# meyerls/FruitNeRF

Measured on AMD Instinct MI355X. Metric: train rays/sec, fruit_nerf on synthetic apple 800x800, higher is better.
Workload: dtype f32 fwd (MLP GEMMs: 3-piece bf16 split, 6 products, ~2^-24) / 2-piece bwd (dX, dW: 3 products, ~2^-17; its forward recompute 3-piece); everything else f32

## Files before the change

fruitnerf_amd/csrc/field_bf16.hpp:

```cpp
#pragma once
#include "field_layers.hpp"

namespace fnr {

using bf16x8 = __attribute__((ext_vector_type(8))) __bf16;
using f32x8 = __attribute__((ext_vector_type(8))) float;

enum { MLP_FP32 = 0, MLP_BF16 = 1, MLP_BF16X3 = 3 };

template <class Cfg>
struct BfImage {
  static constexpr int NL = Cfg::NLAYERS;
  static constexpr int nib_used(int l) { return l == Cfg::L_COL0 ? Cfg::HB : Cfg::nib(l); }
  static constexpr int nkb(int l) { return (nib_used(l) + 1) / 2; }
  static constexpr int nkbT(int l) { return (Cfg::nob(l) + 1) / 2; }
  static constexpr bool hasT(int l) { return l != Cfg::L_SEM0; }
  static constexpr int fblocks(int l) { return Cfg::nob(l) * nkb(l); }
  static constexpr int tblocks(int l) { return hasT(l) ? nib_used(l) * nkbT(l) : 0; }
  static constexpr int foff(int l) {
    int o = 0;
    for (int i = 0; i < l; ++i) o += fblocks(i);
    return o;
  }
  static constexpr int F_TOTAL = foff(NL);
// ... 87 lines not shown
    pack_field_weights_block<Cfg>(p, packed, b);
    return;
  }
  b -= nb_pack;
  if (b < nb_pack16) {
    pack_field_weights_bf16_block<Cfg>(p, ns, image, b);
    return;
  }
  b -= nb_pack16;
  color_ray_bias_block<Cfg, true>(p, nullptr, rays, embedding, mean_embedding, ray_bias, b,
                                  (int)gridDim.x - nb_pack - nb_pack16);
}
template <class Cfg>
static inline void launch_prepare_field(const FieldPtrs& p, float* packed, int ns, __bf16* image, const RaysDev& rays,
                                        const float* embedding, const float* mean_embedding, float* ray_bias,
                                        hipStream_t st) {
  const int nb_pack = pack_field_weights_blocks<Cfg>();
  const int nb_pack16 = ns > 0 ? pack_field_weights_bf16_blocks<Cfg>() : 0;
  const long long nb_bias = color_ray_bias_blocks(rays);
  hipLaunchKernelGGL((k_prepare_field<Cfg>), dim3((unsigned)(nb_pack + nb_pack16 + nb_bias)), dim3(256), 0, st, p, packed, ns,
                     image, rays, embedding, mean_embedding, ray_bias, nb_pack, nb_pack16);
}

template <class Cfg, class Segs, int NS>
struct BfLds {
  using Img = BfImage<Cfg>;
  static constexpr int blocks(int s) { return Segs::isT(s) ? Img::tblocks(Segs::layer(s)) : Img::fblocks(Segs::layer(s)); }
  static constexpr int off(int s) {
    int o = 0;
    for (int i = 0; i < s; ++i) o += blocks(i) * NS;
    return o;
  }
  static constexpr int FRAGS = off(Segs::N);
  static constexpr int BYTES = FRAGS * 1024;
  static constexpr int find(int layer, bool isT) {
    for (int i = 0; i < Segs::N; ++i)
      if (Segs::layer(i) == layer && Segs::isT(i) == isT) return i;
    return -1;
  }
  template <int LAYER, bool IS_T>
  __device__ static __forceinline__ const bf16x8* seg(const bf16x8* lds) {
    constexpr int s = find(LAYER, IS_T);
    static_assert(s >= 0, "layer not staged by this kernel");
    return lds + off(s) * 64;
  }
  template <int LAYER, bool IS_T>
  static constexpr int seg_blocks() { return blocks(find(LAYER, IS_T)); }
  static constexpr int chunk_begin(int c) { return off(c / NS) * 64 + (c % NS) * blocks(c / NS) * 64; }
  static constexpr long long chunk_src(int c) {
    const int s = c / NS, pc = c % NS;
    return (long long)pc * Img::BLOCKS * 64 + (Segs::isT(s) ? Img::toff(Segs::layer(s)) : Img::foff(Segs::layer(s))) * 64;
  }
  template <int THREADS>
  __device__ static __forceinline__ void stage(bf16x8* __restrict__ lds, const __bf16* __restrict__ image) {
    constexpr int T = FRAGS * 64, NCH = Segs::N * NS;
    constexpr int PER = (T + THREADS - 1) / THREADS;
    static_assert(PER <= 32, "staging batch too large");
    const f32x4* img = reinterpret_cast<const f32x4*>(image);
    f32x4* dst = reinterpret_cast<f32x4*>(lds);
    f32x4 v[PER];
#pragma unroll
    for (int u = 0; u < PER; ++u) {
      const int f = (int)threadIdx.x + u * THREADS;
      long long delta = chunk_src(0) - chunk_begin(0);
#pragma unroll
      for (int c = 1; c < NCH; ++c) delta = (f >= chunk_begin(c)) ? chunk_src(c) - chunk_begin(c) : delta;
      if (f < T) v[u] = img[f + delta];
    }
#pragma unroll
    for (int u = 0; u < PER; ++u) {
      const int f = (int)threadIdx.x + u * THREADS;
      if (f < T) dst[f] = v[u];
    }
  }
};

template <class Cfg, int L, int NS, int THREADS>
__device__ __forceinline__ void bf_build_T(bf16x8* __restrict__ lds, const float* __restrict__ packed) {
  constexpr int NIB = Cfg::nib(L), NKT = (Cfg::nob(L) + 1) / 2, TB = NIB * NKT;
  for (int idx = threadIdx.x; idx < TB * 64; idx += THREADS) {
    const int blk = idx >> 6, lane = idx & 63;
    const int i = lane & 15, g = lane >> 4;
    const int kb = blk % NKT, ib = blk / NKT;
    float w[8];
#pragma unroll
    for (int e = 0; e < 8; ++e) {
      const int ob = 2 * kb + (e >> 2), row = 4 * g + (e & 3);
      w[e] = ob < Cfg::nob(L) ? packed[Cfg::woff(L) + ((ob * NIB + ib) * 64 + swz_slot(row, i >> 2)) * 4 + (i & 3)] : 0.0f;
    }
#pragma unroll
    for (int pc = 0; pc < NS; ++pc) {
      bf16x8 v;
#pragma unroll
      for (int e = 0; e < 8; ++e) v[e] = bf_piece(w[e], pc);
      lds[pc * TB * 64 + idx] = v;
    }
  }
}

using bf_f32x2 = __attribute__((ext_vector_type(2))) float;
using bf_bf16x2 = __attribute__((ext_vector_type(2))) __bf16;
__device__ __forceinline__ unsigned cvt_pk_bf16(float lo, float hi) {
  const bf_f32x2 v = {lo, hi};
  return __builtin_bit_cast(unsigned, __builtin_convertvector(v, bf_bf16x2));
}
using bf_u32x4 = __attribute__((ext_vector_type(4))) unsigned;
template <int NS>
__device__ __forceinline__ void bf_split(const f32x8 v, bf16x8 (&p)[NS]) {
  bf_u32x4 out[NS];
#pragma unroll
  for (int d = 0; d < 4; ++d) {
    float a = v[2 * d], b = v[2 * d + 1];
#pragma unroll
    for (int pc = 0; pc < NS; ++pc) {
      const unsigned w = cvt_pk_bf16(a, b);
      out[pc][d] = w;
      if (pc + 1 < NS) {
        a -= __builtin_bit_cast(float, w << 16);
        b -= __builtin_bit_cast(float, w & 0xffff0000u);
      }
    }
  }
#pragma unroll
  for (int pc = 0; pc < NS; ++pc) p[pc] = __builtin_bit_cast(bf16x8, out[pc]);
}
template <int NS>
// ... 101 lines not shown
#pragma unroll
    for (int s = NS - 1; s >= 0; --s)
#pragma unroll
      for (int pw = 0; pw <= s; ++pw)
        o[ob] = __builtin_amdgcn_mfma_f32_16x16x32_bf16(w[t & 1][pw], x[kb][s - pw], o[ob], 0, 0, 0);
    __builtin_amdgcn_sched_barrier(0);
  }
}
template <int NS, int NOB, int NIB>
__device__ __forceinline__ void bf_layer1(const bf16x8* __restrict__ seg, const float* __restrict__ B,
                                          const f32x4 (&in)[NIB], f32x4 (&o)[NOB], int lane) {
  const int g = lane >> 4;
#pragma unroll
  for (int ob = 0; ob < NOB; ++ob) o[ob] = *reinterpret_cast<const f32x4*>(B + 16 * ob + 4 * g);
  bf16x8 x[(NIB + 1) / 2][NS];
  bf_operand<NS, NIB>(in, x);
  bf_layer_acc1<NS, NOB, (NIB + 1) / 2>(seg, x, o, lane);
}
template <int NS, int NIBO, int NOB>
__device__ __forceinline__ void bf_layer_T1(const bf16x8* __restrict__ segT, const f32x4 (&G)[NOB], f32x4 (&o)[NIBO],
                                            int lane) {
#pragma unroll
  for (int ib = 0; ib < NIBO; ++ib) o[ib] = f32x4{0.f, 0.f, 0.f, 0.f};
  bf16x8 x[(NOB + 1) / 2][NS];
  bf_operand<NS, NOB>(G, x);
  bf_layer_acc1<NS, NIBO, (NOB + 1) / 2>(segT, x, o, lane);
}

size_t field_bf16_image_bytes();
int field_mlp_fwd_bf16(int cfg, int mode, const FieldPtrs& p, const float* packed, void* image_ws, const float* ray_bias,
                       const RaysDev& rd, int S, long long N, const float2* feats, const uint8_t* selector, float* density,
                       float* rgb, float* logit, float* geo_out, float* h_buf, hipStream_t st);
int field_mlp_fwd_sem_big_bf16(int mode, const FieldPtrs& p, void* image_ws, const float* packed, long long N,
                               const float* h_buf, float* logit, hipStream_t st);
int field_mlp_bwd_sem_big_bf16(int mode, const FieldPtrs& p, void* image_ws, const float* packed, long long N,
                               const float* h_saved, const float* d_logit, float* partials, long long blocks,
                               hipStream_t st, float* d_h_semgrad = nullptr);
namespace pw {
struct BwdArgs {
  const float* packed;
  const __bf16* image;
  const float* ray_bias;
  RaysDev rd;
  int S;
  long long N;
  const float2* feats;
  const float* h_saved;
  const uint8_t* selector;
  const float *d_density, *d_rgb, *d_logit;
  float2* d_feats;
  float *d_h, *gsum_tile, *gsum_extra, *partials;
  long long blocks;
  hipStream_t st;
};
}
int field_mlp_bwd_pw(int cfg, int mode, int branch, const pw::BwdArgs& a, const float2* jac, float4* d_pos);

}
```

fruitnerf_amd/csrc/field_layers.hpp:

```cpp
#pragma once
#include "common.hpp"

namespace fnr {

using f32x4 = __attribute__((ext_vector_type(4))) float;

enum KMap : int { KM_LINEAR = 0, KM_HASH = 1, KM_GEO = 2, KM_COLOR = 3 };

struct FieldCfgBase {
  static constexpr int GEO = 15, HB = 1, NSEM = 2, SEMB = 4;
  static constexpr int NLAYERS = 8;
  enum { L_BASE0 = 0, L_BASE1 = 1, L_SEM0 = 2, L_SEM1 = 3, L_SEM2 = -1, L_HEAD = 4, L_COL0 = 5, L_COL1 = 6, L_COL2 = 7 };
  static constexpr int nob(int l) { constexpr int a[NLAYERS] = {4, 1, 4, 4, 1, 4, 4, 1}; return a[l]; }
  static constexpr int nib(int l) { constexpr int a[NLAYERS] = {2, 4, 1, 4, 4, 4, 4, 4}; return a[l]; }
  static constexpr int out_dim(int l) { constexpr int a[NLAYERS] = {64, 16, 64, 64, 1, 64, 64, 3}; return a[l]; }
  static constexpr int in_dim(int l) { constexpr int a[NLAYERS] = {32, 64, 15, 64, 64, 63, 64, 64}; return a[l]; }
  static constexpr int km(int l) {
    constexpr int a[NLAYERS] = {KM_HASH, KM_LINEAR, KM_GEO, KM_LINEAR, KM_LINEAR, KM_COLOR, KM_LINEAR, KM_LINEAR};
    return a[l];
  }
  static constexpr int woff(int l) {
    int o = 0;
    for (int i = 0; i < l; ++i) o += nob(i) * nib(i) * 256;
    return o;
// ... 252 lines not shown
  float b;
  if constexpr (FROM_RAW) {
    constexpr int IN = Cfg::in_dim(Cfg::L_COL0);
    for (int i = threadIdx.x; i < COLOR_CONST_K * 64; i += 256) {
      const int o = i / COLOR_CONST_K, k = i - o * COLOR_CONST_K;
      Wt[k][o] = p.w[Cfg::L_COL0][o * IN + color_const_col<Cfg>(k)];
    }
    b = p.b[Cfg::L_COL0][lane];
  } else {
    const float* src = packed + Cfg::LDS_FLOATS;
    for (int i = threadIdx.x; i < COLOR_CONST_K * 64; i += 256) Wt[i >> 6][i & 63] = src[i];
    b = packed[Cfg::W_TOTAL + Cfg::boff(Cfg::L_COL0) + lane];
  }
  __syncthreads();
  for (long long ray = (long long)block * 4 + wave; ray < rays.n_rays; ray += (long long)n_blocks * 4) {
    float c[16];
    sh16_all(rays.directions + 3 * ray, c);
    const float* emb = mean_embedding ? mean_embedding : embedding + (size_t)rays.cam[ray] * 32;
    float e[32];
#pragma unroll
    for (int k = 0; k < 32; k += 4) {
      const f32x4 v = *reinterpret_cast<const f32x4*>(emb + k);
      e[k] = v[0], e[k + 1] = v[1], e[k + 2] = v[2], e[k + 3] = v[3];
    }
    float acc = b;
#pragma unroll
    for (int k = 0; k < 16; ++k) acc = fmaf(Wt[k][lane], c[k], acc);
#pragma unroll
    for (int k = 0; k < 32; ++k) acc = fmaf(Wt[16 + k][lane], e[k], acc);
    ray_bias[(size_t)ray * 64 + lane] = acc;
  }
}
template <class Cfg>
__global__ __launch_bounds__(256) void k_color_ray_bias(const float* __restrict__ packed, RaysDev rays,
                                                        const float* __restrict__ embedding,
                                                        const float* __restrict__ mean_embedding,
                                                        float* __restrict__ ray_bias) {
  FieldPtrs none{};
  color_ray_bias_block<Cfg, false>(none, packed, rays, embedding, mean_embedding, ray_bias, blockIdx.x, gridDim.x);
}
static inline long long color_ray_bias_blocks(const RaysDev& rays) {
  long long blocks = (rays.n_rays + 7) / 8;
  if (blocks > 8ll * device_cu_count()) blocks = 8ll * device_cu_count();
  return blocks < 1 ? 1 : blocks;
}

template <class Cfg>
static inline void launch_color_ray_bias(const float* packed, const RaysDev& rays, const float* embedding,
                                         const float* mean_embedding, float* ray_bias, hipStream_t st) {
  hipLaunchKernelGGL((k_color_ray_bias<Cfg>), dim3((unsigned)color_ray_bias_blocks(rays)), dim3(256), 0, st, packed, rays,
                     embedding, mean_embedding, ray_bias);
}

}
```

fruitnerf_amd/csrc/field_mlp_bwd.hip:

```cpp
#include "field_layers.hpp"
#include "field_bf16.hpp"
#include "sequencer.hpp"

namespace fnr {

enum { BR_COLOR = 0, BR_SEM = 1, BR_BASE = 2, BR_SEM_A = 3, BR_SEM_B = 4 };

constexpr int SCR_LD = 20;
constexpr int SCR_FLOATS = 2 * 64 * SCR_LD;

__device__ __forceinline__ void wave_lds_fence() {
  __builtin_amdgcn_s_waitcnt(0xc07f);
  __builtin_amdgcn_wave_barrier();
  asm volatile("" ::: "memory");
  __builtin_amdgcn_sched_barrier(0);
}

template <int NOB, int NIB_TOTAL, int IB0, int NIBO>
__device__ __forceinline__ void mlp_layer_T(const float* __restrict__ P, const f32x4 (&G)[NOB], f32x4 (&out)[NIBO],
                                            int lane) {
  const int ip = lane & 15, kg = lane >> 4;
  const int a = ip >> 2, b = ip & 3;
  constexpr int QC = (NIBO > 2) ? 2 : NIBO;
  static_assert(NIBO % QC == 0, "input blocks must split evenly");
// ... 557 lines not shown
    for (; b + 7 * RD_Y < nblocks; b += 8 * RD_Y) {
      float v[8];
#pragma unroll
      for (int u = 0; u < 8; ++u) v[u] = partials[(size_t)(b + u * RD_Y) * TOT + idx];
#pragma unroll
      for (int u = 0; u < 8; ++u) s += v[u];
    }
    for (; b < nblocks; b += RD_Y) s += partials[(size_t)b * TOT + idx];
  }
  s_part[y][t] = s;
  __syncthreads();
  if (y != 0 || idx >= TOT) return;
#pragma unroll
  for (int q = 1; q < RD_Y; ++q) s += s_part[q][t];
  if (!ADAM && s == 0.0f) return;
  if (idx < Cfg::W_TOTAL) {
    int l = 0;
#pragma unroll
    for (int q = 1; q < Cfg::NLAYERS; ++q)
      if (idx >= Cfg::woff(q)) l = q;
    const int local = idx - Cfg::woff(l);
    const int r = local & 3, slot = (local >> 2) & 63, blk = local >> 8;
    const int nib = Cfg::nib(l);
    const int ib = blk % nib, ob = blk / nib;
    const int g = slot >> 4, i = (slot & 15) ^ g;
    const int out = 16 * ob + i;
    const int col = kmap<Cfg>(Cfg::km(l), ib, g, r, Cfg::in_dim(l));
    if (out < Cfg::out_dim(l) && col >= 0) {
      float* dst = const_cast<float*>(grads.w[l]) + out * Cfg::in_dim(l) + col;
      if constexpr (ADAM) weight_adam_entry(wa, dst, s);
      else *dst += s;
    }
  } else {
    const int bi = idx - Cfg::W_TOTAL;
    int l = 0;
#pragma unroll
    for (int q = 1; q < Cfg::NLAYERS; ++q)
      if (bi >= Cfg::boff(q)) l = q;
    const int o = bi - Cfg::boff(l);
    if (o < Cfg::out_dim(l)) {
      float* dst = const_cast<float*>(grads.b[l]) + o;
      if constexpr (ADAM) weight_adam_entry(wa, dst, s);
      else *dst += s;
    }
  }
}

template <class Cfg, bool ADAM>
__global__ __launch_bounds__(RD_IDX * RD_Y) void k_reduce_dw(const float* __restrict__ partials, int nblocks, FieldPtrs grads,
                                                             WeightAdam wa) {
  reduce_dw_block<Cfg, ADAM>((int)blockIdx.x, partials, nblocks, grads, wa);
}

constexpr int RAYG_RB = 16;
template <class Cfg>
__global__ __launch_bounds__(256) void k_color_ray_grads(RaysDev rays, int S, long long N,
                                                         const float* __restrict__ embedding,
                                                         const float* __restrict__ gsum_tile,
                                                         const float* __restrict__ gsum_extra,
                                                         float* __restrict__ g_ray, float* __restrict__ partials) {
  __shared__ float Gs[RAYG_RB][64];
  __shared__ __attribute__((aligned(16))) float Cs[RAYG_RB][COLOR_CONST_K];
  const int t = threadIdx.x, o = t & 63, kq = t >> 6;
  const long long R = rays.n_rays;
  f32x4 acc[3];
  float accb = 0.0f;
#pragma unroll
  for (int q = 0; q < 3; ++q) acc[q] = f32x4{0.f, 0.f, 0.f, 0.f};
  for (long long base = (long long)blockIdx.x * RAYG_RB; base < R; base += (long long)gridDim.x * RAYG_RB) {
#pragma unroll
    for (int i = 0; i < RAYG_RB / 4; ++i) {
      const int rr = kq + 4 * i;
      const long long ray = base + rr;
      float v = 0.0f;
      if (ray < R) {
        const long long s_lo = ray * S, s_hi = s_lo + S;
        for (long long tl = s_lo >> 4; tl <= (s_hi - 1) >> 4; ++tl) {
          const long long first = 16 * tl, last = (16 * tl + 15 < N) ? 16 * tl + 15 : N - 1;
          if (first >= s_lo && last < s_hi) v += gsum_tile[(size_t)tl * 64 + o];
        }
        if (gsum_extra) v += gsum_extra[(size_t)ray * 64 + o];
        g_ray[(size_t)ray * 64 + o] = v;
      }
      Gs[rr][o] = v;
    }
#pragma unroll
    for (int u = 0; u < RAYG_RB * COLOR_CONST_K / 256; ++u) {
      const int idx = t + 256 * u;
      const int rr = idx / COLOR_CONST_K, k = idx - rr * COLOR_CONST_K;
      const long long ray = base + rr;
      float v = 0.0f;
      if (ray < R) {
        if (k < 16) {
          float c[16];
          sh16_all(rays.directions + 3 * ray, c);
#pragma unroll
          for (int q = 0; q < 16; ++q) v = (k == q) ? c[q] : v;
        } else {
          v = embedding[(size_t)rays.cam[ray] * 32 + (k - 16)];
        }
      }
      Cs[rr][k] = v;
    }
    __syncthreads();
#pragma unroll
    for (int rr = 0; rr < RAYG_RB; ++rr) {
      const float gv = Gs[rr][o];
      const f32x4* cr = reinterpret_cast<const f32x4*>(&Cs[rr][12 * kq]);
#pragma unroll
      for (int q = 0; q < 3; ++q) {
        const f32x4 cv = cr[q];
#pragma unroll
        for (int e = 0; e < 4; ++e) acc[q][e] = fmaf(gv, cv[e], acc[q][e]);
      }
      accb += gv;
    }
    __syncthreads();
  }
  float* part = partials + (size_t)blockIdx.x * (Cfg::W_TOTAL + Cfg::B_TOTAL);
  const int ob = o >> 4, i = o & 15;
  constexpr int NIB0 = Cfg::HB + 3;
#pragma unroll
  for (int q = 0; q < 12; ++q) {
    const int k = 12 * kq + q, ib = Cfg::HB + (k >> 4), kk = k & 15;
    part[Cfg::woff(Cfg::L_COL0) + ((ob * NIB0 + ib) * 64 + swz_slot(i, kk >> 2)) * 4 + (kk & 3)] = acc[q >> 2][q & 3];
  }
  if (kq == 0) part[Cfg::W_TOTAL + Cfg::boff(Cfg::L_COL0) + o] = accb;
}
static_assert(RAYG_RB * COLOR_CONST_K % 256 == 0, "staging loop covers the batch exactly");

template <class Cfg, bool ADAM>
__device__ __forceinline__ void embedding_grad_block(int c, const RaysDev& rays, const float* __restrict__ g_ray,
                                                     const float* __restrict__ packed, float* __restrict__ g_embedding,
                                                     const WeightAdam& wa) {
  __shared__ float red[16][64];
  const int lane = threadIdx.x & 63, wave = threadIdx.x >> 6;
  float acc = 0.0f;
  for (long long base = 64 * wave; base < rays.n_rays; base += 1024) {
    const long long r = base + lane;
    unsigned long long match = __ballot(r < rays.n_rays && rays.cam[r] == c);
    while (match) {
      const int bit = __builtin_ctzll(match);
      match &= match - 1;
      acc += g_ray[(size_t)(base + bit) * 64 + lane];
    }
  }
  red[wave][lane] = acc;
  __syncthreads();
  if (threadIdx.x < 64) {
    float s = 0.0f;
#pragma unroll
    for (int w = 0; w < 16; ++w) s += red[w][lane];
    red[0][lane] = s;
  }
  __syncthreads();
  const int k = threadIdx.x >> 5, oo = threadIdx.x & 31;
  const float* Wt = packed + Cfg::LDS_FLOATS + (16 + k) * 64;
  float s = fmaf(Wt[oo], red[0][oo], Wt[oo + 32] * red[0][oo + 32]);
#pragma unroll
  for (int m = 16; m >= 1; m >>= 1) s += __shfl_xor(s, m, 64);
  if constexpr (ADAM) {
    if (oo == 0) weight_adam_entry(wa, g_embedding + (size_t)c * 32 + k, s);
  } else {
    if (oo == 0 && s != 0.0f) g_embedding[(size_t)c * 32 + k] += s;
  }
}

template <class Cfg, bool ADAM>
__global__ __launch_bounds__(1024) void k_embedding_grad(RaysDev rays, const float* __restrict__ g_ray,
                                                         const float* __restrict__ packed,
                                                         float* __restrict__ g_embedding, WeightAdam wa) {
  embedding_grad_block<Cfg, ADAM>((int)blockIdx.x, rays, g_ray, packed, g_embedding, wa);
}

static_assert(RD_IDX * RD_Y == 1024, "k_finish_weights: both roles are 1024-thread workgroups");
template <class Cfg, bool ADAM>
__global__ __launch_bounds__(1024) void k_finish_weights(int n_images, RaysDev rays, const float* __restrict__ g_ray,
                                                         const float* __restrict__ packed, float* __restrict__ g_embedding,
                                                         const float* __restrict__ partials, int nblocks, FieldPtrs grads,
                                                         WeightAdam wa) {
  if ((int)blockIdx.x < n_images) embedding_grad_block<Cfg, ADAM>((int)blockIdx.x, rays, g_ray, packed, g_embedding, wa);
  else reduce_dw_block<Cfg, ADAM>((int)blockIdx.x - n_images, partials, nblocks, grads, wa);
// ... 37 lines not shown

template <class Cfg>
int field_mlp_bwd_launch(const FieldPtrs& p, const FieldPtrs& gp, const fnr_field_net* net, const fnr_field_net* grads,
                         const RaysDev& rd, int S, long long N, const float* feats, const float* h_saved,
                         const float* ray_bias_saved, const float* packed_saved, const uint8_t* selector,
                         const float* d_density, const float* d_rgb, const float* d_logit, float* d_feats,
                         const BwdWorkspace& ws, hipStream_t st, const float* jacobian = nullptr,
                         float* d_position = nullptr, const WeightAdam* wadam = nullptr, bool semgrad = false) {
  const float2* jac = reinterpret_cast<const float2*>(jacobian);
  float4* d_pos = reinterpret_cast<float4*>(d_position);
  const long long n_tiles = (N + 15) / 16;
  const long long max_blocks = device_cu_count();
  float* partials = ws.partials;
  float* packed = ws.packed;
  float* gsum_extra = (S % 16 != 0) ? ws.gsum_extra : nullptr;
  const float2* f2 = reinterpret_cast<const float2*>(feats);
  float2* df2 = reinterpret_cast<float2*>(d_feats);
  void* bf16_image = ws.bf16_image;
  if (packed_saved) {
    packed = const_cast<float*>(packed_saved);
    bf16_image = reinterpret_cast<char*>(packed) + field_fwd_ws_image_offset();
  } else {
    launch_pack_field_weights<Cfg>(p, packed, st);
    FNR_LAUNCH_CHECK();
  }
  const float* ray_bias = ray_bias_saved;
  if (!ray_bias) {
    launch_color_ray_bias<Cfg>(packed, rd, net->embedding, nullptr, ws.ray_bias, st);
    FNR_LAUNCH_CHECK();
    ray_bias = ws.ray_bias;
  }
  if (gsum_extra) FNR_HIP(hipMemsetAsync(gsum_extra, 0, (size_t)rd.n_rays * 64 * sizeof(float), st));
  long long blocks = (n_tiles + 3) / 4;
  if (blocks > max_blocks) blocks = max_blocks;
  const dim3 grid((unsigned)blocks);
  const int mode = net->mlp_mode;
  constexpr int cfg_id = Cfg::NSEM == 2 ? 0 : 1;
  const bool bf_all = mode != FNR_MLP_FP32;
  const bool bf_sem_big = mode != FNR_MLP_FP32 && Cfg::NSEM == 3;
  const pw::BwdArgs bf{packed, reinterpret_cast<const __bf16*>(bf16_image), ray_bias, rd, S, N, f2, h_saved, selector, d_density,
                       d_rgb, d_logit, df2, ws.d_h, ws.gsum_tile, gsum_extra, partials, blocks, st};
  if (bf_all) {
    if (!packed_saved) {
      launch_pack_field_weights_bf16<Cfg>(p, mode == FNR_MLP_BF16 ? 1 : 3, reinterpret_cast<__bf16*>(bf16_image), st);
      FNR_LAUNCH_CHECK();
    }
    const int rc = field_mlp_bwd_pw(cfg_id, mode, 0, bf, nullptr, nullptr);
    if (rc) return rc;
  } else {
    hipLaunchKernelGGL((k_field_mlp_bwd_color<Cfg, 8>), grid, dim3(512), 0, st, packed, ray_bias, rd, S, N, h_saved, d_rgb,
                       ws.d_h, ws.gsum_tile, gsum_extra, partials);
  }
  FNR_LAUNCH_CHECK();
  {
    long long rb = (rd.n_rays + RAYG_RB - 1) / RAYG_RB;
    if (rb > blocks) rb = blocks;
    hipLaunchKernelGGL((k_color_ray_grads<Cfg>), dim3((unsigned)rb), dim3(256), 0, st, rd, S, N, net->embedding,
                       ws.gsum_tile, gsum_extra, ws.g_ray, partials);
    FNR_LAUNCH_CHECK();
  }
  if (bf_sem_big) {
    int rc = field_mlp_bwd_sem_big_bf16(mode, p, bf16_image, packed, N, h_saved, d_logit, partials, blocks, st,
                                        semgrad ? ws.d_h : nullptr);
    if (rc) return rc;
    rc = field_mlp_bwd_pw(cfg_id, mode, 2, bf, jac, d_pos);
    if (rc) return rc;
  } else if (bf_all) {
    int rc = semgrad ? field_mlp_bwd_pw(cfg_id, mode, 3, bf, nullptr, nullptr) : FNR_OK;
    if (rc) return rc;
    rc = field_mlp_bwd_pw(cfg_id, mode, 1, bf, nullptr, nullptr);
    if (rc) return rc;
    rc = field_mlp_bwd_pw(cfg_id, mode, 2, bf, jac, d_pos);
    if (rc) return rc;
  } else if constexpr (Cfg::NSEM == 2) {
    if (semgrad)
      hipLaunchKernelGGL((k_field_mlp_bwd_sem<Cfg, 8, true, float*>), grid, dim3(512), 0, st, packed, N, h_saved, d_logit,
                         partials, ws.d_h);
    else
      hipLaunchKernelGGL((k_field_mlp_bwd_sem<Cfg, 8>), grid, dim3(512), 0, st, packed, N, h_saved, d_logit, partials);
    FNR_LAUNCH_CHECK();
  } else {
    if (semgrad)
      hipLaunchKernelGGL((k_field_mlp_bwd_sem_big<Cfg, true, 4, true, float*>), grid, dim3(256), 0, st, packed, N, h_saved,
                         d_logit, partials, ws.d_h);
    else
      hipLaunchKernelGGL((k_field_mlp_bwd_sem_big<Cfg, true, 4>), grid, dim3(256), 0, st, packed, N, h_saved, d_logit,
                         partials);
    FNR_LAUNCH_CHECK();
    hipLaunchKernelGGL((k_field_mlp_bwd_sem_big<Cfg, false, 4>), grid, dim3(256), 0, st, packed, N, h_saved, d_logit,
                       partials);
    FNR_LAUNCH_CHECK();
  }
  if (!bf_all) {
    hipLaunchKernelGGL((k_field_mlp_bwd_base<Cfg, 8>), grid, dim3(512), 0, st, packed, N, f2, selector, d_density, ws.d_h,
                       df2, partials);
    FNR_LAUNCH_CHECK();
  }
  constexpr int TOT = Cfg::W_TOTAL + Cfg::B_TOTAL;
  const unsigned finish_blocks = (unsigned)net->n_images + (unsigned)((TOT + RD_IDX - 1) / RD_IDX);
  if (wadam)
    hipLaunchKernelGGL((k_finish_weights<Cfg, true>), dim3(finish_blocks), dim3(1024), 0, st, (int)net->n_images, rd, ws.g_ray,
                       packed, grads->embedding, partials, (int)blocks, gp, *wadam);
  else
    hipLaunchKernelGGL((k_finish_weights<Cfg, false>), dim3(finish_blocks), dim3(1024), 0, st, (int)net->n_images, rd,
                       ws.g_ray, packed, grads->embedding, partials, (int)blocks, gp, WeightAdam{});
  FNR_LAUNCH_CHECK();
  if (jac && d_pos && !bf_all) return position_contract(N, net->grid.n_levels, jac, df2, d_pos, st);
  return FNR_OK;
}
}

extern "C" size_t fnr_field_mlp_bwd_workspace_bytes(int64_t n_rays, int S) {
  if (n_rays < 0 || S <= 0) return 0;
  return bwd_workspace(nullptr, n_rays, S).bytes;
}

static int field_mlp_bwd_entry(const fnr_field_net* net, const fnr_field_net* grads, const fnr_rays* rays, int S,
                                 const float* feats, const float* h_saved, const float* ray_bias_saved,
                                 const float* packed_saved, const uint8_t* selector, const float* d_density, const float* d_rgb, const float* d_logit, float* d_feats,
                                 void* workspace, size_t workspace_bytes, void* stream, const float* jacobian,
                               float* d_position, const fnr_table_adam* weight_adam = nullptr,
                               const float* grad_arena = nullptr, bool semgrad = false) {
  WeightAdam wa{};
// ... 109 lines not shown
```

fruitnerf_amd/csrc/field_mlp_bwd_pw.hip:

```cpp
#include <type_traits>

#include "field_bf16.hpp"

namespace fnr {
namespace pw {

using s16x4 = __attribute__((ext_vector_type(4))) short;
using s16x8 = __attribute__((ext_vector_type(8))) short;
using u32x4 = __attribute__((ext_vector_type(4))) unsigned;
typedef s16x4 __attribute__((address_space(3))) lds_s16x4;

constexpr int TILE_BYTES = 512;
template <int NS, int NT>
constexpr int scratch_bytes() { return 4 * NS * NT * TILE_BYTES; }

template <int NT, int NB>
struct Acts {
  f32x4 v[NT][NB];
};
template <int NT, int NB, int NS>
struct Ops {
  bf16x8 v[NT][(NB + 1) / 2][NS];
};
template <int NT, int NB, int NS>
// ... 465 lines not shown
          const int ray = first_ray[t] + (j - col);
#pragma unroll
          for (int ob = 0; ob < 4; ++ob)
#pragma unroll
            for (int r = 0; r < 4; ++r) atomicAdd(&gsum_extra[(size_t)ray * 64 + 16 * ob + 4 * g + r], rs[0][ob][r]);
        }
      }
    }
    Acts<NT, HB> Gh;
    layer<NT, NS, HB, 4>(T::template seg<LC0, true>(wt), nullptr, g1, Gh, lane);
#pragma unroll
    for (int t = 0; t < NT; ++t)
      if (sm.ok[t]) {
#pragma unroll
        for (int hb = 0; hb < HB; ++hb) *reinterpret_cast<f32x4*>(d_h + (size_t)sm.n[t] * (16 * HB) + 16 * hb + 4 * g) = Gh.v[t][hb];
      }
  }
  const int lane = lane0;
  float* part = partials + (size_t)blockIdx.x * (Cfg::W_TOTAL + Cfg::B_TOTAL);
  constexpr int NA = 4 * HB, NALL = NA + 25;
  struct Table {
    __device__ static __forceinline__ Dest get(int b) {
      constexpr int NA = 4 * Cfg::HB;
      if (b < NA) return Dest{Cfg::woff(LC0), b / Cfg::HB, b % Cfg::HB, Cfg::HB + 3, 0};
      b -= NA;
      if (b < 16) return Dest{Cfg::woff(LC1), b >> 2, b & 3, 4, 0};
      if (b < 20) return Dest{Cfg::woff(LC2), 0, b - 16, 4, 0};
      if (b < 24) return Dest{Cfg::W_TOTAL + Cfg::boff(LC1), b - 20, 0, 0, 1};
      return Dest{Cfg::W_TOTAL + Cfg::boff(LC2), 0, 0, 0, 1};
    }
  };
  f32x4 all[NALL];
#pragma unroll
  for (int i = 0; i < NA; ++i) all[i] = accA[i];
#pragma unroll
  for (int i = 0; i < 16; ++i) all[NA + i] = accB[i];
#pragma unroll
  for (int i = 0; i < 4; ++i) all[NA + 16 + i] = accC[i];
#pragma unroll
  for (int i = 0; i < 4; ++i) all[NA + 20 + i] = bias_total(bB[i]);
  all[NA + 24] = bias_total(bC[0]);
  reduce_and_store<NALL, WAVES, Table>(smem, part, all, wave, lane);
  constexpr int NIB0 = Cfg::HB + 3;
  for (int i = threadIdx.x; i < 4 * 3 * 256; i += THREADS) {
    const int blk = i >> 8, ob = blk / 3, ib = Cfg::HB + blk % 3;
    part[Cfg::woff(LC0) + (ob * NIB0 + ib) * 256 + (i & 255)] = 0.0f;
  }
  for (int i = threadIdx.x; i < 64; i += THREADS) part[Cfg::W_TOTAL + Cfg::boff(LC0) + i] = 0.0f;
}

template <class Cfg, int NSF, int NS, int NT, int WAVES>
__global__ __launch_bounds__(64 * WAVES, WAVES / 4) void k_field_mlp_bwd_sem_pw(
    const float* __restrict__ packed, const __bf16* __restrict__ image, int N, const float* __restrict__ h_saved,
    const float* __restrict__ d_logit, float* __restrict__ partials) {
  static_assert(Cfg::NSEM == 2 && Cfg::HB == 1, "`fruit_nerf` shape");
  constexpr int THREADS = 64 * WAVES;
  constexpr int LS0 = Cfg::L_SEM0, LS1 = Cfg::L_SEM1, LH = Cfg::L_HEAD;
  static_assert(LS1 == LS0 + 1 && LH == LS1 + 1, "the branch's layers are adjacent in the fp32 image");
  using L = Lds<Cfg, SegsSemF<Cfg>, SegsSemT<Cfg>, NSF, NS, NT, WAVES, 128>;
  using F = typename L::F;
  using T = typename L::T;
  extern __shared__ __attribute__((aligned(16))) unsigned char smem[];
  bf16x8* wf = reinterpret_cast<bf16x8*>(smem);
  bf16x8* wt = reinterpret_cast<bf16x8*>(smem + F::BYTES);
  float* fbias = reinterpret_cast<float*>(smem + L::FB_OFF);
  F::template stage<THREADS>(wf, image);
  T::template stage<THREADS>(wt, image);
  for (int i = threadIdx.x; i < 128; i += THREADS) fbias[i] = packed[Cfg::W_TOTAL + Cfg::boff(LS0) + i];
  __syncthreads();
  const int lane0 = threadIdx.x & 63, wave = threadIdx.x >> 6;
  unsigned char* scr = smem + L::SCR_OFF + wave * scratch_bytes<NS, NT>();
  f32x4 accH[4], accB[16], accA[4];
  f32x4 bH[1], bB[4], bA[4];
  zero_vec(accH);
  zero_vec(accB);
  zero_vec(accA);
  zero_vec(bH);
  zero_vec(bB);
  zero_vec(bA);
  const int n_groups = (N + 16 * NT - 1) / (16 * NT);
  for (int gr = blockIdx.x * WAVES + wave; gr < n_groups; gr += gridDim.x * WAVES) {
    asm volatile("" ::: "memory");
    int lane = lane0;
    asm volatile("" : "+v"(lane));
    const int j = lane & 15, g = lane >> 4;
    const Samples<NT> sm(gr, j, N);
    Ops<NT, 4, NSF> x1;
    Ops<NT, 4, NS> x2;
    {
      Ops<NT, 1, NSF> hx;
      Acts<NT, 1> h;
      Acts<NT, 4> s1;
#pragma unroll
      for (int t = 0; t < NT; ++t) h.v[t][0] = *reinterpret_cast<const f32x4*>(h_saved + (size_t)sm.n[t] * 16 + 4 * g);
      to_ops(hx, h);
      layer<NT, NSF, 4, 1>(F::template seg<LS0, false>(wf), fbias, hx, s1, lane);
      relu(s1);
      to_ops(x1, s1);
    }
    {
      Acts<NT, 4> s2;
      layer<NT, NSF, 4, 4>(F::template seg<LS1, false>(wf), fbias + 64, x1, s2, lane);
      to_ops(x2, s2);
    }
    Ops<NT, 1, NS> gl;
    {
      Acts<NT, 1> Gl;
#pragma unroll
      for (int t = 0; t < NT; ++t) {
        Gl.v[t][0] = f32x4{0.f, 0.f, 0.f, 0.f};
        if (g == 0 && sm.ok[t]) Gl.v[t][0][0] = d_logit[sm.n[t]];
      }
      bias_add(bH, Gl);
      to_ops(gl, Gl);
    }
    dw_round<NT, NS, 1, 4>(scr, gl, x2, accH, lane);
    Ops<NT, 4, NS> g2;
    {
      Acts<NT, 4> Gs2;
      layer<NT, NS, 4, 1>(T::template seg<LH, true>(wt), nullptr, gl, Gs2, lane);
      bias_add(bB, Gs2);
      to_ops(g2, Gs2);
    }
    dw_round<NT, NS, 4, 4>(scr, g2, x1, accB, lane);
    Ops<NT, 4, NS> g1;
    {
      Acts<NT, 4> Gs1;
      layer<NT, NS, 4, 4>(T::template seg<LS1, true>(wt), nullptr, g2, Gs1, lane);
      gate(Gs1, x1);
      bias_add(bA, Gs1);
      to_ops(g1, Gs1);
    }
    {
      Acts<NT, 1> h;
      Ops<NT, 1, NS> hx;
#pragma unroll
      for (int t = 0; t < NT; ++t) h.v[t][0] = *reinterpret_cast<const f32x4*>(h_saved + (size_t)sm.n[t] * 16 + 4 * g);
      to_ops(hx, h);
      dw_round<NT, NS, 4, 1>(scr, g1, hx, accA, lane);
    }
  }
  const int lane = lane0;
  float* part = partials + (size_t)blockIdx.x * (Cfg::W_TOTAL + Cfg::B_TOTAL);
  struct Table {
    __device__ static __forceinline__ Dest get(int b) {
      if (b < 4) return Dest{Cfg::woff(LS0), b, 0, 1, 0};
      if (b < 20) return Dest{Cfg::woff(LS1), (b - 4) >> 2, (b - 4) & 3, 4, 0};
      if (b < 24) return Dest{Cfg::woff(LH), 0, b - 20, 4, 0};
      if (b < 28) return Dest{Cfg::W_TOTAL + Cfg::boff(LS0), b - 24, 0, 0, 1};
      if (b < 32) return Dest{Cfg::W_TOTAL + Cfg::boff(LS1), b - 28, 0, 0, 1};
      return Dest{Cfg::W_TOTAL + Cfg::boff(LH), 0, 0, 0, 1};
    }
  };
  f32x4 all[33];
#pragma unroll
  for (int i = 0; i < 4; ++i) all[i] = accA[i];
#pragma unroll
  for (int i = 0; i < 16; ++i) all[4 + i] = accB[i];
#pragma unroll
  for (int i = 0; i < 4; ++i) all[20 + i] = accH[i];
#pragma unroll
  for (int i = 0; i < 4; ++i) all[24 + i] = bias_total(bA[i]);
#pragma unroll
  for (int i = 0; i < 4; ++i) all[28 + i] = bias_total(bB[i]);
  all[32] = bias_total(bH[0]);
  reduce_and_store<33, WAVES, Table>(smem, part, all, wave, lane);
}

template <class Cfg, int NSF, int NS, int NT, int WAVES, bool POSGRAD>
__global__ __launch_bounds__(64 * WAVES, WAVES / 4) void k_field_mlp_bwd_base_pw(
    const float* __restrict__ packed, const __bf16* __restrict__ image, int N, const float2* __restrict__ feats,
    const float* __restrict__ h_saved, const uint8_t* __restrict__ selector, const float* __restrict__ d_density,
    const float* __restrict__ d_h, float2* __restrict__ d_feats, float* __restrict__ partials,
    const float2* __restrict__ jac, float4* __restrict__ d_pos) {
  constexpr int HB = Cfg::HB;
  static_assert(HB == 1 || HB == 2, "built shapes");
  constexpr int THREADS = 64 * WAVES;
  constexpr int LB0 = Cfg::L_BASE0, LB1 = Cfg::L_BASE1;
  static_assert(LB1 == LB0 + 1, "the branch's layers are adjacent in the fp32 image");
  using L = Lds<Cfg, SegsBaseF<Cfg>, SegsBaseT<Cfg>, NSF, NS, NT, WAVES, 64>;
  using F = typename L::F;
  using T = typename L::T;
  extern __shared__ __attribute__((aligned(16))) unsigned char smem[];
  bf16x8* wf = reinterpret_cast<bf16x8*>(smem);
  bf16x8* wt = reinterpret_cast<bf16x8*>(smem + F::BYTES);
  float* fbias = reinterpret_cast<float*>(smem + L::FB_OFF);
  F::template stage<THREADS>(wf, image);
  T::template stage<THREADS>(wt, image);
  for (int i = threadIdx.x; i < 64; i += THREADS) fbias[i] = packed[Cfg::W_TOTAL + Cfg::boff(LB0) + i];
  __syncthreads();
  const int lane0 = threadIdx.x & 63, wave = threadIdx.x >> 6;
  unsigned char* scr = smem + L::SCR_OFF + wave * scratch_bytes<NS, NT>();
  f32x4 accB[4 * HB], accA[8];
  f32x4 bB[HB], bA[4];
  zero_vec(accB);
  zero_vec(accA);
// ... 233 lines not shown
    const int once = ensure_dyn_lds<kern>(L::BYTES);
    if (once) return once;
    hipLaunchKernelGGL(kern, dim3((unsigned)a.blocks), dim3(THREADS), L::BYTES, a.st, a.packed, a.image, (int)a.N, a.h_saved,
                       a.d_logit, a.d_h);
    FNR_LAUNCH_CHECK();
    return FNR_OK;
  } else {
    FNR_CHECK_ARG(false, "the fruit_nerf_big semantic branch forms its input gradient itself (field_mlp_bwd_sem_big_bf16)");
  }
}
}

namespace pw {
#ifndef FNR_PW_NT_COLOR
#define FNR_PW_NT_COLOR 1
#endif
#ifndef FNR_PW_NT_SEM
#define FNR_PW_NT_SEM 2
#endif
#ifndef FNR_PW_NT_BASE
#define FNR_PW_NT_BASE 2
#endif
#ifndef FNR_PW_NT_BASE_BIG
#define FNR_PW_NT_BASE_BIG 1
#endif
#ifndef FNR_PW_WAVES
#define FNR_PW_WAVES 8
#endif

template <class Cfg, int NSF, int NS>
static int launch(int branch, const BwdArgs& a, const float2* jac, float4* d_pos) {
  if (branch == 3) return pw_dx::launch<Cfg, NSF, NS>(a);
  constexpr int WAVES = FNR_PW_WAVES, THREADS = 64 * WAVES;
  FNR_CHECK_ARG(a.N < (1ll << 31) - 64, "field_mlp_bwd: %lld samples exceed the 32-bit sample index of the backward kernels", a.N);
  const int n = (int)a.N;
  const dim3 grid((unsigned)a.blocks);
  if (branch == 0) {
    constexpr int NT = FNR_PW_NT_COLOR;
    using L = Lds<Cfg, SegsColF<Cfg>, SegsColT<Cfg>, NSF, NS, NT, WAVES, 80>;
    static_assert(L::BYTES <= 160 * 1024, "colour branch exceeds the LDS");
    constexpr auto kern = k_field_mlp_bwd_color_pw<Cfg, NSF, NS, NT, WAVES>;
    const int once = ensure_dyn_lds<kern>(L::BYTES);
    if (once) return once;
    hipLaunchKernelGGL(kern, grid, dim3(THREADS), L::BYTES, a.st, a.packed, a.image, a.ray_bias, a.rd, a.S, n, a.h_saved, a.d_rgb,
                       a.d_h, a.gsum_tile, a.gsum_extra, a.partials);
  } else if (branch == 1) {
    if constexpr (Cfg::NSEM == 2) {
      constexpr int NT = NSF == 1 ? 1 : FNR_PW_NT_SEM;
      using L = Lds<Cfg, SegsSemF<Cfg>, SegsSemT<Cfg>, NSF, NS, NT, WAVES, 128>;
      static_assert(L::BYTES <= 160 * 1024, "semantic branch exceeds the LDS");
      constexpr auto kern = k_field_mlp_bwd_sem_pw<Cfg, NSF, NS, NT, WAVES>;
      const int once = ensure_dyn_lds<kern>(L::BYTES);
      if (once) return once;
      hipLaunchKernelGGL(kern, grid, dim3(THREADS), L::BYTES, a.st, a.packed, a.image, n, a.h_saved, a.d_logit, a.partials);
    } else {
      FNR_CHECK_ARG(false, "the fruit_nerf_big semantic branch has its own kernel (field_mlp_bwd_sem_big_bf16)");
    }
  } else {
    constexpr int NT = Cfg::HB == 1 ? FNR_PW_NT_BASE : FNR_PW_NT_BASE_BIG;
    using L = Lds<Cfg, SegsBaseF<Cfg>, SegsBaseT<Cfg>, NSF, NS, NT, WAVES, 64>;
    static_assert(L::BYTES <= 160 * 1024, "base branch exceeds the LDS");
    if (jac && d_pos) {
      constexpr auto kern = k_field_mlp_bwd_base_pw<Cfg, NSF, NS, NT, WAVES, true>;
      const int once = ensure_dyn_lds<kern>(L::BYTES);
      if (once) return once;
      hipLaunchKernelGGL(kern, grid, dim3(THREADS), L::BYTES, a.st, a.packed, a.image, n, a.feats, a.h_saved, a.selector,
                         a.d_density, a.d_h, a.d_feats, a.partials, jac, d_pos);
    } else {
      constexpr auto kern = k_field_mlp_bwd_base_pw<Cfg, NSF, NS, NT, WAVES, false>;
      const int once = ensure_dyn_lds<kern>(L::BYTES);
      if (once) return once;
      hipLaunchKernelGGL(kern, grid, dim3(THREADS), L::BYTES, a.st, a.packed, a.image, n, a.feats, a.h_saved, a.selector,
                         a.d_density, a.d_h, a.d_feats, a.partials, jac, d_pos);
    }
  }
  FNR_LAUNCH_CHECK();
  return FNR_OK;
}

}

int field_mlp_bwd_pw(int cfg, int mode, int branch, const pw::BwdArgs& a, const float2* jac, float4* d_pos) {
#define FNR_PW_LAUNCH(C, A, B) pw::launch<C, A, B>(branch, a, jac, d_pos)
  if (cfg == 0) return mode == MLP_BF16 ? FNR_PW_LAUNCH(FieldCfgBase, 1, 1) : FNR_PW_LAUNCH(FieldCfgBase, 3, 2);
  return mode == MLP_BF16 ? FNR_PW_LAUNCH(FieldCfgBig, 1, 1) : FNR_PW_LAUNCH(FieldCfgBig, 3, 2);
#undef FNR_PW_LAUNCH
}

}
```

Measured before the change: 6.368 million.

## Fuse per-ray colour gradient reduction into the semantic backward kernel as a rider

The standalone k_color_ray_grads kernel is folded into the semantic-branch backward kernel. The first ray_blocks workgroups run the per-ray gsum reduction and colour-layer-0 weight accumulation in the transposition scratch LDS before the MLP work starts. Their ray loads are interleaved with the weight-image staging loads to hide latency. The tile-range loop is also rewritten as closed-form first/last bounds with chunked loads. This removes one kernel launch and its tail, at the cost of extra registers and serial work in the rider blocks, which may now finish later than the rest.

```diff
diff --git a/fruitnerf_amd/csrc/field_bf16.hpp b/fruitnerf_amd/csrc/field_bf16.hpp
--- a/fruitnerf_amd/csrc/field_bf16.hpp
+++ b/fruitnerf_amd/csrc/field_bf16.hpp
@@ -163,13 +163,13 @@
     return (long long)pc * Img::BLOCKS * 64 + (Segs::isT(s) ? Img::toff(Segs::layer(s)) : Img::foff(Segs::layer(s))) * 64;
   }
   template <int THREADS>
-  __device__ static __forceinline__ void stage(bf16x8* __restrict__ lds, const __bf16* __restrict__ image) {
+  static constexpr int stage_per() { return (FRAGS * 64 + THREADS - 1) / THREADS; }
+  template <int THREADS>
+  __device__ static __forceinline__ void stage_load(const __bf16* __restrict__ image, f32x4 (&v)[stage_per<THREADS>()]) {
     constexpr int T = FRAGS * 64, NCH = Segs::N * NS;
-    constexpr int PER = (T + THREADS - 1) / THREADS;
+    constexpr int PER = stage_per<THREADS>();
     static_assert(PER <= 32, "staging batch too large");
     const f32x4* img = reinterpret_cast<const f32x4*>(image);
-    f32x4* dst = reinterpret_cast<f32x4*>(lds);
-    f32x4 v[PER];
 #pragma unroll
     for (int u = 0; u < PER; ++u) {
       const int f = (int)threadIdx.x + u * THREADS;
@@ -178,11 +178,22 @@
       for (int c = 1; c < NCH; ++c) delta = (f >= chunk_begin(c)) ? chunk_src(c) - chunk_begin(c) : delta;
       if (f < T) v[u] = img[f + delta];
     }
-#pragma unroll
-    for (int u = 0; u < PER; ++u) {
+  }
+  template <int THREADS>
+  __device__ static __forceinline__ void stage_store(bf16x8* __restrict__ lds, const f32x4 (&v)[stage_per<THREADS>()]) {
+    constexpr int T = FRAGS * 64;
+    f32x4* dst = reinterpret_cast<f32x4*>(lds);
+#pragma unroll
+    for (int u = 0; u < stage_per<THREADS>(); ++u) {
       const int f = (int)threadIdx.x + u * THREADS;
       if (f < T) dst[f] = v[u];
     }
+  }
+  template <int THREADS>
+  __device__ static __forceinline__ void stage(bf16x8* __restrict__ lds, const __bf16* __restrict__ image) {
+    f32x4 v[stage_per<THREADS>()];
+    stage_load<THREADS>(image, v);
+    stage_store<THREADS>(lds, v);
   }
 };
 
@@ -390,6 +401,9 @@
   float *d_h, *gsum_tile, *gsum_extra, *partials;
   long long blocks;
   hipStream_t st;
+  long long ray_blocks = 0;
+  const float* embedding = nullptr;
+  float* g_ray = nullptr;
 };
 }
 int field_mlp_bwd_pw(int cfg, int mode, int branch, const pw::BwdArgs& a, const float2* jac, float4* d_pos);
diff --git a/fruitnerf_amd/csrc/field_layers.hpp b/fruitnerf_amd/csrc/field_layers.hpp
--- a/fruitnerf_amd/csrc/field_layers.hpp
+++ b/fruitnerf_amd/csrc/field_layers.hpp
@@ -328,4 +328,113 @@
                      embedding, mean_embedding, ray_bias);
 }
 
-}
+constexpr int RAYG_RB = 16;
+template <class Cfg>
+struct ColorRayGrads {
+  static constexpr int PER_G = RAYG_RB / 4, PER_C = RAYG_RB * COLOR_CONST_K / 256;
+  static_assert(RAYG_RB * COLOR_CONST_K % 256 == 0, "the park step covers the batch exactly");
+  static constexpr int GS_FLOATS = RAYG_RB * 64, LDS_FLOATS = GS_FLOATS + RAYG_RB * COLOR_CONST_K;
+  f32x4 acc[3];
+  float accb;
+  float gv[PER_G], cv[PER_C];
+  __device__ __forceinline__ void init() {
+#pragma unroll
+    for (int q = 0; q < 3; ++q) acc[q] = f32x4{0.f, 0.f, 0.f, 0.f};
+    accb = 0.0f;
+  }
+  __device__ __forceinline__ void load(long long base, const RaysDev& rays, int S, long long N,
+                                       const float* __restrict__ embedding, const float* __restrict__ gsum_tile,
+                                       const float* __restrict__ gsum_extra, float* __restrict__ g_ray, int t) {
+    const int o = t & 63, kq = t >> 6;
+    const long long R = rays.n_rays;
+#pragma unroll
+    for (int u = 0; u < PER_C; ++u) {
+      const int idx = t + 256 * u;
+      const int rr = idx / COLOR_CONST_K;
+      int k = idx - rr * COLOR_CONST_K;
+      asm volatile("" : "+v"(k));
+      const long long ray = base + rr, rc = ray < R ? ray : R - 1;
+      const float e = embedding[(size_t)rays.cam[rc] * 32 + (k < 16 ? 0 : k - 16)];
+      float c[16];
+      sh16_all(rays.directions + 3 * rc, c);
+      float v = e;
+#pragma unroll
+      for (int q = 0; q < 16; ++q) v = (k == q) ? c[q] : v;
+      cv[u] = ray < R ? v : 0.0f;
+    }
+    const float* tp[PER_G];
+    int n_in[PER_G];
+    float xe[PER_G];
+#pragma unroll
+    for (int i = 0; i < PER_G; ++i) {
+      const long long ray = base + kq + 4 * i;
+      const long long s_lo = ray * S, s_hi = s_lo + S;
+      const long long t_lo = s_lo >> 4, t_hi = (s_hi - 1) >> 4;
+      const long long first_in = (s_lo & 15) ? t_lo + 1 : t_lo;
+      const long long end = (16 * t_hi + 15 < N) ? 16 * t_hi + 15 : N - 1;
+      const long long last_in = end < s_hi ? t_hi : t_hi - 1;
+      const long long n = last_in - first_in + 1;
+      n_in[i] = (ray < R && n > 0) ? (int)n : 0;
+      tp[i] = gsum_tile + (size_t)first_in * 64 + o;
+      xe[i] = (gsum_extra && ray < R) ? gsum_extra[(size_t)ray * 64 + o] : 0.0f;
+      gv[i] = 0.0f;
+    }
+    constexpr int CH = 4;
+    const int n_over = ((S + 14) >> 4) + 1;
+    for (int c0 = 0; c0 < n_over; c0 += CH) {
+      float x[PER_G][CH];
+#pragma unroll
+      for (int i = 0; i < PER_G; ++i)
+#pragma unroll
+        for (int q = 0; q < CH; ++q) x[i][q] = (c0 + q < n_in[i]) ? tp[i][(size_t)(c0 + q) * 64] : 0.0f;
+#pragma unroll
+      for (int i = 0; i < PER_G; ++i)
+#pragma unroll
+        for (int q = 0; q < CH; ++q)
+          if (c0 + q < n_in[i]) gv[i] += x[i][q];
+    }
+#pragma unroll
+    for (int i = 0; i < PER_G; ++i) {
+      const long long ray = base + kq + 4 * i;
+      if (ray < R) {
+        if (gsum_extra) gv[i] += xe[i];
+        g_ray[(size_t)ray * 64 + o] = gv[i];
+      }
+    }
+  }
+  __device__ __forceinline__ void park(float* __restrict__ Gs, float* __restrict__ Cs, int t) const {
+    const int o = t & 63, kq = t >> 6;
+#pragma unroll
+    for (int i = 0; i < PER_G; ++i) Gs[(kq + 4 * i) * 64 + o] = gv[i];
+#pragma unroll
+    for (int u = 0; u < PER_C; ++u) Cs[t + 256 * u] = cv[u];
+  }
+  __device__ __forceinline__ void accumulate(const float* __restrict__ Gs, const float* __restrict__ Cs, int t) {
+    const int o = t & 63, kq = t >> 6;
+#pragma unroll
+    for (int rr = 0; rr < RAYG_RB; ++rr) {
+      const float g = Gs[rr * 64 + o];
+      const f32x4* cr = reinterpret_cast<const f32x4*>(Cs + rr * COLOR_CONST_K + 12 * kq);
+#pragma unroll
+      for (int q = 0; q < 3; ++q) {
+        const f32x4 c = cr[q];
+#pragma unroll
+        for (int e = 0; e < 4; ++e) acc[q][e] = fmaf(g, c[e], acc[q][e]);
+      }
+      accb += g;
+    }
+  }
+  __device__ __forceinline__ void store(float* __restrict__ part, int t) const {
+    const int o = t & 63, kq = t >> 6;
+    const int ob = o >> 4, i = o & 15;
+    constexpr int NIB0 = Cfg::HB + 3;
+#pragma unroll
+    for (int q = 0; q < 12; ++q) {
+      const int k = 12 * kq + q, ib = Cfg::HB + (k >> 4), kk = k & 15;
+      part[Cfg::woff(Cfg::L_COL0) + ((ob * NIB0 + ib) * 64 + swz_slot(i, kk >> 2)) * 4 + (kk & 3)] = acc[q >> 2][q & 3];
+    }
+    if (kq == 0) part[Cfg::W_TOTAL + Cfg::boff(Cfg::L_COL0) + o] = accb;
+  }
+};
+
+}
diff --git a/fruitnerf_amd/csrc/field_mlp_bwd.hip b/fruitnerf_amd/csrc/field_mlp_bwd.hip
--- a/fruitnerf_amd/csrc/field_mlp_bwd.hip
+++ b/fruitnerf_amd/csrc/field_mlp_bwd.hip
@@ -633,82 +633,26 @@
   reduce_dw_block<Cfg, ADAM>((int)blockIdx.x, partials, nblocks, grads, wa);
 }
 
-constexpr int RAYG_RB = 16;
 template <class Cfg>
 __global__ __launch_bounds__(256) void k_color_ray_grads(RaysDev rays, int S, long long N,
                                                          const float* __restrict__ embedding,
                                                          const float* __restrict__ gsum_tile,
                                                          const float* __restrict__ gsum_extra,
                                                          float* __restrict__ g_ray, float* __restrict__ partials) {
-  __shared__ float Gs[RAYG_RB][64];
-  __shared__ __attribute__((aligned(16))) float Cs[RAYG_RB][COLOR_CONST_K];
-  const int t = threadIdx.x, o = t & 63, kq = t >> 6;
-  const long long R = rays.n_rays;
-  f32x4 acc[3];
-  float accb = 0.0f;
-#pragma unroll
-  for (int q = 0; q < 3; ++q) acc[q] = f32x4{0.f, 0.f, 0.f, 0.f};
-  for (long long base = (long long)blockIdx.x * RAYG_RB; base < R; base += (long long)gridDim.x * RAYG_RB) {
-#pragma unroll
-    for (int i = 0; i < RAYG_RB / 4; ++i) {
-      const int rr = kq + 4 * i;
-      const long long ray = base + rr;
-      float v = 0.0f;
-      if (ray < R) {
-        const long long s_lo = ray * S, s_hi = s_lo + S;
-        for (long long tl = s_lo >> 4; tl <= (s_hi - 1) >> 4; ++tl) {
-          const long long first = 16 * tl, last = (16 * tl + 15 < N) ? 16 * tl + 15 : N - 1;
-          if (first >= s_lo && last < s_hi) v += gsum_tile[(size_t)tl * 64 + o];
-        }
-        if (gsum_extra) v += gsum_extra[(size_t)ray * 64 + o];
-        g_ray[(size_t)ray * 64 + o] = v;
-      }
-      Gs[rr][o] = v;
-    }
-#pragma unroll
-    for (int u = 0; u < RAYG_RB * COLOR_CONST_K / 256; ++u) {
-      const int idx = t + 256 * u;
-      const int rr = idx / COLOR_CONST_K, k = idx - rr * COLOR_CONST_K;
-      const long long ray = base + rr;
-      float v = 0.0f;
-      if (ray < R) {
-        if (k < 16) {
-          float c[16];
-          sh16_all(rays.directions + 3 * ray, c);
-#pragma unroll
-          for (int q = 0; q < 16; ++q) v = (k == q) ? c[q] : v;
-        } else {
-          v = embedding[(size_t)rays.cam[ray] * 32 + (k - 16)];
-        }
-      }
-      Cs[rr][k] = v;
-    }
+  __shared__ __attribute__((aligned(16))) float lds[ColorRayGrads<Cfg>::LDS_FLOATS];
+  float *Gs = lds, *Cs = lds + ColorRayGrads<Cfg>::GS_FLOATS;
+  const int t = threadIdx.x;
+  ColorRayGrads<Cfg> c;
+  c.init();
+  for (long long base = (long long)blockIdx.x * RAYG_RB; base < rays.n_rays; base += (long long)gridDim.x * RAYG_RB) {
+    c.load(base, rays, S, N, embedding, gsum_tile, gsum_extra, g_ray, t);
+    c.park(Gs, Cs, t);
     __syncthreads();
-#pragma unroll
-    for (int rr = 0; rr < RAYG_RB; ++rr) {
-      const float gv = Gs[rr][o];
-      const f32x4* cr = reinterpret_cast<const f32x4*>(&Cs[rr][12 * kq]);
-#pragma unroll
-      for (int q = 0; q < 3; ++q) {
-        const f32x4 cv = cr[q];
-#pragma unroll
-        for (int e = 0; e < 4; ++e) acc[q][e] = fmaf(gv, cv[e], acc[q][e]);
-      }
-      accb += gv;
-    }
+    c.accumulate(Gs, Cs, t);
     __syncthreads();
   }
-  float* part = partials + (size_t)blockIdx.x * (Cfg::W_TOTAL + Cfg::B_TOTAL);
-  const int ob = o >> 4, i = o & 15;
-  constexpr int NIB0 = Cfg::HB + 3;
-#pragma unroll
-  for (int q = 0; q < 12; ++q) {
-    const int k = 12 * kq + q, ib = Cfg::HB + (k >> 4), kk = k & 15;
-    part[Cfg::woff(Cfg::L_COL0) + ((ob * NIB0 + ib) * 64 + swz_slot(i, kk >> 2)) * 4 + (kk & 3)] = acc[q >> 2][q & 3];
-  }
-  if (kq == 0) part[Cfg::W_TOTAL + Cfg::boff(Cfg::L_COL0) + o] = accb;
-}
-static_assert(RAYG_RB * COLOR_CONST_K % 256 == 0, "staging loop covers the batch exactly");
+  c.store(partials + (size_t)blockIdx.x * (Cfg::W_TOTAL + Cfg::B_TOTAL), t);
+}
 
 template <class Cfg, bool ADAM>
 __device__ __forceinline__ void embedding_grad_block(int c, const RaysDev& rays, const float* __restrict__ g_ray,
@@ -852,9 +796,11 @@
                        ws.d_h, ws.gsum_tile, gsum_extra, partials);
   }
   FNR_LAUNCH_CHECK();
-  {
-    long long rb = (rd.n_rays + RAYG_RB - 1) / RAYG_RB;
-    if (rb > blocks) rb = blocks;
+  long long rb = (rd.n_rays + RAYG_RB - 1) / RAYG_RB;
+  if (rb > blocks) rb = blocks;
+  const char* ride_env = getenv("FNR_COLOR_RAYS_RIDE");
+  const bool rays_ride = !(ride_env && ride_env[0] == '0' && !ride_env[1]) && bf_all && !bf_sem_big && !semgrad;
+  if (!rays_ride) {
     hipLaunchKernelGGL((k_color_ray_grads<Cfg>), dim3((unsigned)rb), dim3(256), 0, st, rd, S, N, net->embedding,
                        ws.gsum_tile, gsum_extra, ws.g_ray, partials);
     FNR_LAUNCH_CHECK();
@@ -868,7 +814,9 @@
   } else if (bf_all) {
     int rc = semgrad ? field_mlp_bwd_pw(cfg_id, mode, 3, bf, nullptr, nullptr) : FNR_OK;
     if (rc) return rc;
-    rc = field_mlp_bwd_pw(cfg_id, mode, 1, bf, nullptr, nullptr);
+    pw::BwdArgs sem = bf;
+    if (rays_ride) sem.ray_blocks = rb, sem.embedding = net->embedding, sem.g_ray = ws.g_ray;
+    rc = field_mlp_bwd_pw(cfg_id, mode, 1, sem, nullptr, nullptr);
     if (rc) return rc;
     rc = field_mlp_bwd_pw(cfg_id, mode, 2, bf, jac, d_pos);
     if (rc) return rc;
diff --git a/fruitnerf_amd/csrc/field_mlp_bwd_pw.hip b/fruitnerf_amd/csrc/field_mlp_bwd_pw.hip
--- a/fruitnerf_amd/csrc/field_mlp_bwd_pw.hip
+++ b/fruitnerf_amd/csrc/field_mlp_bwd_pw.hip
@@ -541,9 +541,12 @@
 template <class Cfg, int NSF, int NS, int NT, int WAVES>
 __global__ __launch_bounds__(64 * WAVES, WAVES / 4) void k_field_mlp_bwd_sem_pw(
     const float* __restrict__ packed, const __bf16* __restrict__ image, int N, const float* __restrict__ h_saved,
-    const float* __restrict__ d_logit, float* __restrict__ partials) {
+    const float* __restrict__ d_logit, float* __restrict__ partials, RaysDev rays, int S,
+    const float* __restrict__ embedding, const float* __restrict__ gsum_tile, const float* __restrict__ gsum_extra,
+    float* __restrict__ g_ray, int ray_blocks) {
   static_assert(Cfg::NSEM == 2 && Cfg::HB == 1, "`fruit_nerf` shape");
   constexpr int THREADS = 64 * WAVES;
+  static_assert(THREADS >= 256, "the rider's thread mapping");
   constexpr int LS0 = Cfg::L_SEM0, LS1 = Cfg::L_SEM1, LH = Cfg::L_HEAD;
   static_assert(LS1 == LS0 + 1 && LH == LS1 + 1, "the branch's layers are adjacent in the fp32 image");
   using L = Lds<Cfg, SegsSemF<Cfg>, SegsSemT<Cfg>, NSF, NS, NT, WAVES, 128>;
@@ -553,10 +556,44 @@
   bf16x8* wf = reinterpret_cast<bf16x8*>(smem);
   bf16x8* wt = reinterpret_cast<bf16x8*>(smem + F::BYTES);
   float* fbias = reinterpret_cast<float*>(smem + L::FB_OFF);
-  F::template stage<THREADS>(wf, image);
-  T::template stage<THREADS>(wt, image);
+  float* part = partials + (size_t)blockIdx.x * (Cfg::W_TOTAL + Cfg::B_TOTAL);
+  using Ray = ColorRayGrads<Cfg>;
+  static_assert(Ray::LDS_FLOATS * 4 <= WAVES * scratch_bytes<NS, NT>() && L::SCR_OFF % 16 == 0, "Gs / Cs fit the transposition region");
+  float* Gs = reinterpret_cast<float*>(smem + L::SCR_OFF);
+  float* Cs = Gs + Ray::GS_FLOATS;
+  const bool rider = (int)blockIdx.x < ray_blocks;
+  const bool ray_thread = rider && threadIdx.x < 256;
+  const int rt = threadIdx.x;
+  Ray rg;
+  long long ray_base = (long long)blockIdx.x * RAYG_RB;
+  {
+    f32x4 vf[F::template stage_per<THREADS>()], vt[T::template stage_per<THREADS>()];
+    F::template stage_load<THREADS>(image, vf);
+    T::template stage_load<THREADS>(image, vt);
+    if (ray_thread) {
+      rg.init();
+      rg.load(ray_base, rays, S, N, embedding, gsum_tile, gsum_extra, g_ray, rt);
+    }
+    F::template stage_store<THREADS>(wf, vf);
+    T::template stage_store<THREADS>(wt, vt);
+  }
   for (int i = threadIdx.x; i < 128; i += THREADS) fbias[i] = packed[Cfg::W_TOTAL + Cfg::boff(LS0) + i];
+  if (ray_thread) rg.park(Gs, Cs, rt);
   __syncthreads();
+  if (rider) {
+    for (;;) {
+      if (ray_thread) rg.accumulate(Gs, Cs, rt);
+      __syncthreads();
+      ray_base += (long long)ray_blocks * RAYG_RB;
+      if (ray_base >= rays.n_rays) break;
+      if (ray_thread) {
+        rg.load(ray_base, rays, S, N, embedding, gsum_tile, gsum_extra, g_ray, rt);
+        rg.park(Gs, Cs, rt);
+      }
+      __syncthreads();
+    }
+    if (ray_thread) rg.store(part, rt);
+  }
   const int lane0 = threadIdx.x & 63, wave = threadIdx.x >> 6;
   unsigned char* scr = smem + L::SCR_OFF + wave * scratch_bytes<NS, NT>();
   f32x4 accH[4], accB[16], accA[4];
@@ -630,7 +667,6 @@
     }
   }
   const int lane = lane0;
-  float* part = partials + (size_t)blockIdx.x * (Cfg::W_TOTAL + Cfg::B_TOTAL);
   struct Table {
     __device__ static __forceinline__ Dest get(int b) {
       if (b < 4) return Dest{Cfg::woff(LS0), b, 0, 1, 0};
@@ -970,7 +1006,11 @@
       constexpr auto kern = k_field_mlp_bwd_sem_pw<Cfg, NSF, NS, NT, WAVES>;
       const int once = ensure_dyn_lds<kern>(L::BYTES);
       if (once) return once;
-      hipLaunchKernelGGL(kern, grid, dim3(THREADS), L::BYTES, a.st, a.packed, a.image, n, a.h_saved, a.d_logit, a.partials);
+      FNR_CHECK_ARG(a.ray_blocks >= 0 && a.ray_blocks <= a.blocks && a.ray_blocks <= (a.rd.n_rays + RAYG_RB - 1) / RAYG_RB &&
+                        (a.ray_blocks == 0 || (a.embedding && a.g_ray && a.gsum_tile)),
+                    "field_mlp_bwd: the semantic branch's rider needs a partial image and a batch of rays per workgroup");
+      hipLaunchKernelGGL(kern, grid, dim3(THREADS), L::BYTES, a.st, a.packed, a.image, n, a.h_saved, a.d_logit, a.partials, a.rd,
+                         a.S, a.embedding, a.gsum_tile, a.gsum_extra, a.g_ray, (int)a.ray_blocks);
     } else {
       FNR_CHECK_ARG(false, "the fruit_nerf_big semantic branch has its own kernel (field_mlp_bwd_sem_big_bf16)");
     }
```

Measured after the change: 6.401 million (median of 6 runs). About the same (+0.5%).
